# KPU-AGC/ipcr

Hardware: AMD Instinct MI355X
Metric: genome Gbases scanned/sec (k=2) (higher is better)
Workload: dtype u32

## Files before the change

### ipcr_amd/csrc/host.cpp

```cpp
#include "ipcr_hip.h"

#include <emmintrin.h>
#include <immintrin.h>
#include <sched.h>
#include <sys/prctl.h>
#include <time.h>
#include <unistd.h>
#include <dlfcn.h>
#include <hip/hip_runtime_api.h>
#include <hsa/hsa.h>
#include <hsa/hsa_ext_amd.h>

#include <algorithm>
#include <array>
#include <atomic>
#include <chrono>
#include <condition_variable>
#include <functional>
#include <cstdarg>
#include <cstdio>
#include <cstdlib>
#include <cstring>
#include <map>
#include <memory>
// ... 1788 lines not shown
        e = hipMemcpyAsync(c->d_bad, c->h_bad, 8, hipMemcpyHostToDevice, c->st);
        if (e == hipSuccess) e = hipMemcpyAsync(c->d_sites, c->h_sites, m * sizeof(ipcr_site_dev), hipMemcpyHostToDevice, c->st);
        if (e == hipSuccess) e = ipcr::launch_read_sites(c->st, g->planes, g->rst, c->d_sites, (uint32_t)m, c->d_out, g->d_exc, nruns, c->d_bad);
        if (e == hipSuccess) e = hipMemcpyAsync(out + offsets[i0], c->d_out, bytes, hipMemcpyDeviceToHost, c->st);
        if (e == hipSuccess) e = hipMemcpyAsync(c->h_bad, c->d_bad, 8, hipMemcpyDeviceToHost, c->st);
        if (e == hipSuccess) e = hipStreamSynchronize(c->st);
        if (e == hipSuccess && *c->h_bad != ~0ull) {
            const unsigned long long v = *c->h_bad;
            const int64_t i = i0 + (int64_t)(v >> 16);
            const unsigned off = (unsigned)((v >> 8) & 0xFFu), b = (unsigned)(v & 0xFFu);
            st = fail(IPCR_ERR_PRIMER, "%s: site %lld (record %d, position %lld): byte 0x%02x%s%c%s has no reverse complement "
                      "(upper-case IUPAC DNA only, core/primer/rc.go:8-24)", what, (long long)i, sites[i].record, (long long)sites[i].pos + off, b,
                      (b >= 0x21 && b < 0x7F) ? " '" : "", (b >= 0x21 && b < 0x7F) ? (char)b : ' ', (b >= 0x21 && b < 0x7F) ? "'" : "");
        }
        i0 += (int64_t)m;
    }
    read_ctx_release(c);
    if (st != IPCR_OK) return st;
    HIPCHK(e);
    return IPCR_OK;
}
}

extern "C" {

ipcr_status ipcr_genome_read_sites(const ipcr_genome *cg, const ipcr_site *sites, int64_t n, uint8_t *out, uint64_t cap,
                                   uint64_t *offsets, uint64_t *needed) {
    if (!cg || n < 0 || (n && !sites) || !offsets || !needed) return fail(IPCR_ERR_INVALID, "ipcr_genome_read_sites: null argument");
    return read_sites("ipcr_genome_read_sites", const_cast<ipcr_genome *>(cg), sites, n, out, cap, offsets, needed);
}

uint64_t ipcr_genome_exception_runs(const ipcr_genome *cg) {
    if (!cg) return 0;
    ipcr_genome *g = const_cast<ipcr_genome *>(cg);
    DeviceGuard dg(g->device);
    std::lock_guard<std::mutex> lk(g->read_mu);
    if (genome_finalize(g) != IPCR_OK) return 0;
    return (g->exc_dropped || !g->exc_capture) ? UINT64_MAX : g->exc_sorted;
}

uint32_t ipcr_genome_num_records(const ipcr_genome *g) { return g ? (uint32_t)g->rec_start.size() : 0; }
uint64_t ipcr_genome_record_len(const ipcr_genome *g, uint32_t r) { return (g && r < g->rec_len.size()) ? g->rec_len[r] : 0; }
const char *ipcr_genome_record_id(const ipcr_genome *g, uint32_t r) { return (g && r < g->ids.size()) ? g->ids[r].c_str() : ""; }
uint64_t ipcr_genome_total_bases(const ipcr_genome *g) { return g ? g->total_bases : 0; }
uint64_t ipcr_genome_tile_bytes(const ipcr_genome *g) {
    return g ? ((g->next_col + 63) / 64) * IPCR_BLOCK_PLANE_WORDS * 4ull : 0;
}
double ipcr_genome_pack_ms(const ipcr_genome *g) { return g ? g->pack_ms : 0; }

uint8_t ipcr_genome_record_flags(const ipcr_genome *g, uint32_t record) {
    if (!g || record >= g->rec_start.size()) return 0;
    if (!g->flags_valid) {
        DeviceGuard dg(g->device);
        if (genome_finalize(const_cast<ipcr_genome *>(g)) != IPCR_OK) return 0;
    }
    return (uint8_t)((g->flags[record] & 1u) | (genome_any_reset(g) ? 2u : 0u));
}

}


struct ipcr_scratch {
    const ipcr_panel *panel = nullptr;
    int device = 0;
    SetDev *sdev[2] = {nullptr, nullptr};
    hipStream_t stream = nullptr;
    hipEvent_t ev[4] = {nullptr, nullptr, nullptr, nullptr};
    ipcr_queue_entry *d_queue = nullptr;
    uint64_t qcap = 0;
    unsigned long long *d_qcounts = nullptr;
    uint64_t prefix_hint = 256;
    ipcr_hit_rec *d_hits = nullptr;
    uint64_t hcap = 0;
    unsigned long long *d_counts = nullptr;
    void *d_hitbuf = nullptr;
    uint32_t cset = 0;
    struct Lane {
        hipStream_t s = nullptr;
        ~Lane() { if (s) (void)hipStreamDestroy(s); }
    };
    std::shared_ptr<Lane> own_lane;
    std::shared_ptr<Lane> lane_next;
    std::shared_ptr<Lane> lane_used;
    hipEvent_t ev_done = nullptr;
    hipStream_t cstream = nullptr;
    struct Pending {
        bool active = false, empty = false;
        int mode = 0;
        bool fused = false;
        bool verified = false;
        bool on_lane = false;
        bool published = false;
        bool times_pending = false;
        uint32_t nrec = 0, check_rst = 0, cset_used = 0;
        uint64_t nblocks = 0, pre = 0;
        uint64_t block0 = 0;
        bool segment = false;
        std::chrono::steady_clock::time_point t0;
    } pend;
    void *pinned = nullptr;
    uint32_t *d_tickets = nullptr;
    uint32_t seq = 0;
    uint64_t seg_overflow = 0;
    std::vector<ipcr_hit> hits;
    std::vector<ipcr_hit> hits_raw;
    std::vector<uint32_t> bucket;
    std::vector<ipcr_product> products;
    std::vector<uint64_t> last_rec_len;
    std::vector<uint64_t> last_rec_start;
    ipcr_scan_stats stats{};
    std::vector<ipcr_chunk_window> windows;
    bool products_in_windows = false;
    ipcr_genome *chunk = nullptr;
    bool dev_hits_stale = false;
    bool last_was_chunk = false;
    uint8_t *h_stage[2] = {nullptr, nullptr};
    hipEvent_t ev_stage[2] = {nullptr, nullptr};
    uint8_t *h_planes = nullptr;
    uint64_t h_planes_cap = 0;
    std::shared_ptr<std::atomic<int>> counted_in;
    uint8_t *d_amps = nullptr; uint64_t amps_cap = 0;
    ipcr_genome *nest = nullptr;
    void *d_probe_misc = nullptr; uint64_t probe_misc_cap = 0;
    hipStream_t probe_stream = nullptr;
    uint8_t *h_probe = nullptr; uint64_t h_probe_cap = 0;
    uint32_t probe_tag = 0;
    hipStream_t probe_on = nullptr;
    int64_t probe_pending = -1;
    uint64_t probe_res_off = 0;
};

namespace {

constexpr uint64_t PREFIX_HITS = 65536;
constexpr uint64_t QCAP_INIT = 1ull << 13;
constexpr uint64_t HCAP_INIT = 1ull << 20;
constexpr uint64_t QCAP_MAX = 1ull << 23;
constexpr uint64_t HCAP_MAX = 1ull << 28;
uint64_t hcap_soft() {
    const char *e = getenv("IPCR_TEST_HCAP_SOFT");
    return e && *e ? std::max<uint64_t>(64, strtoull(e, nullptr, 10)) : (1ull << 24);
}

ipcr_status panel_upload(const ipcr_panel *cp, int mode, int slot, SetDev **out) {
    ipcr_panel *p = const_cast<ipcr_panel *>(cp);
    std::lock_guard<std::mutex> lock(p->mu);
    std::unique_ptr<PanelDev> &pd = p->devs[slot];
    if (!pd) { pd.reset(new PanelDev); pd->slot = slot; }
    PatternSet &s = p->set[mode];
    SetDev &d = pd->set[mode];
    *out = &d;
    if (!d.dev && !s.host.empty()) {
        HIPCHK(hipMalloc((void **)&d.dev, s.host.size() * sizeof(ipcr_dev_pattern)));
        HIPCHK(hipMemcpy(d.dev, s.host.data(), s.host.size() * sizeof(ipcr_dev_pattern), hipMemcpyHostToDevice));
    }
    const bool force_index = getenv("IPCR_FORCE_INDEX") && atoi(getenv("IPCR_FORCE_INDEX")) != 0;
    if (p->specialize && !d.jit_tried && !s.host.empty()) {
        d.jit_tried = true;
        static const bool async_on = env_flag("IPCR_JIT_ASYNC", true);
        const bool async = async_on && !force_index && s.host.size() <= 16;
        if (!force_index && !async) {
            d.jit = ipcr::jit_build(s.host, p->cfg.max_mm, s.jit_error);
            d.jit_pub.store(&d.jit, std::memory_order_release);
        } else if (async) {
            d.jit_state.store(1);
            const int max_mm = p->cfg.max_mm;
            SetDev *dp = &d;
            PatternSet *sp = &s;
            d.jit_thread = std::thread([dp, sp, max_mm, slot] {
                DeviceGuard dgt(slot);
                std::string err;
                dp->jit = ipcr::jit_build(sp->host, max_mm, err);
                if (dp->jit.empty()) sp->jit_error = err;
                dp->jit_state.store(2, std::memory_order_release);
            });
        }
// ... 167 lines not shown
    }
    dedup_sorted_hits(out);
}

void trace(const char *what, const void *s) {
    static const bool on = getenv("IPCR_DEBUG_TIMES") != nullptr;
    static const auto t0 = std::chrono::steady_clock::now();
    if (on) fprintf(stderr, "[t %10.1f us] %p %s\n", std::chrono::duration<double, std::micro>(std::chrono::steady_clock::now() - t0).count(), s, what);
}

double ms_since(std::chrono::steady_clock::time_point a) {
    return std::chrono::duration<double, std::milli>(std::chrono::steady_clock::now() - a).count();
}

bool env_flag(const char *name, bool dflt) {
    const char *v = getenv(name);
    return (v && *v) ? atoi(v) != 0 : dflt;
}

uint32_t *pinned_seq(const ipcr_scratch *s) {
    return reinterpret_cast<uint32_t *>(static_cast<char *>(s->pinned) + 64 + PREFIX_HITS * sizeof(ipcr_hit));
}

std::atomic<bool> g_publish_broken{false};

bool publish_enabled() {
    static const bool on = env_flag("IPCR_PUBLISH", true);
    return on && !g_publish_broken.load(std::memory_order_relaxed);
}

ipcr_status wait_published(ipcr_scratch *s) {
    volatile uint32_t *w = pinned_seq(s);
    const uint32_t want = s->seq;
    const hipStream_t lane = s->lane_used ? s->lane_used->s : s->stream;
    const auto t0 = std::chrono::steady_clock::now();
    static const int sleep_us = getenv("IPCR_WAIT_SLEEP_US") ? atoi(getenv("IPCR_WAIT_SLEEP_US")) : 0;
    static const int spin_us = getenv("IPCR_WAIT_SPIN_US") ? atoi(getenv("IPCR_WAIT_SPIN_US")) : 30;
    if (sleep_us > 0) {
        static thread_local bool slack_set = false;
        if (!slack_set) { (void)prctl(PR_SET_TIMERSLACK, 1000UL, 0, 0, 0); slack_set = true; }
    }
    for (uint64_t spin = 1;; ++spin) {
        if (__atomic_load_n(w, __ATOMIC_ACQUIRE) == want) return IPCR_OK;
        if (sleep_us > 0 && (spin & 63u) == 0 && ms_since(t0) * 1000.0 > (double)spin_us) {
            struct timespec ts = {0, sleep_us * 1000L};
            (void)nanosleep(&ts, nullptr);
        }
        if (spin < 0x10000u) __builtin_ia32_pause();
        else std::this_thread::yield();
        if ((spin & 0xFFFFu) == 0) {
            const hipError_t q = hipStreamQuery(lane);
            if (q == hipSuccess) {
                if (__atomic_load_n(w, __ATOMIC_ACQUIRE) == want) return IPCR_OK;
                return IPCR_ERR_UNSUPPORTED;
            }
            if (q != hipErrorNotReady) return fail(IPCR_ERR_DEVICE, "HIP: %s", hipGetErrorString(q));
            if (ms_since(t0) > 120000.0) return fail(IPCR_ERR_DEVICE, "scan did not finish within 120 s");
        }
    }
}

ipcr_status scan_segmented(const ipcr_panel *p, ipcr_scratch *s, ipcr_genome *g, uint64_t seen_hits);
inline bool hit_has_idx_below(const ipcr_hit *h, int tw);

ipcr_status scan_launch(const ipcr_panel *p, ipcr_scratch *s, ipcr_genome *g) {
    ipcr_scratch::Pending &pd = s->pend;
    const PatternSet &set = p->set[pd.mode];
    const SetDev &sd = *s->sdev[pd.mode];
    static const std::vector<ipcr::JitFilter *> none;
    const std::vector<ipcr::JitFilter *> *pub = sd.jit_pub.load(std::memory_order_acquire);
    const std::vector<ipcr::JitFilter *> &jit = pub ? *pub : none;
    const auto te = std::chrono::steady_clock::now();
    unsigned long long *cnt = s->d_counts + 4u * s->cset, *cnt_next = s->d_counts + 4u * (s->cset ^ 1u);
    const uint64_t qset = (uint64_t)IPCR_QUEUE_SHARDS * IPCR_QUEUE_COUNTER_STRIDE;
    unsigned long long *qc = s->d_qcounts + qset * s->cset, *qc_next = s->d_qcounts + qset * (s->cset ^ 1u);
    pd.cset_used = s->cset;
    s->cset ^= 1u;
    const uint64_t nblocks = pd.nblocks, block0 = pd.block0;
    trace("launch>", s);
    const hipStream_t own = s->stream;
    const hipStream_t lane = s->lane_next ? s->lane_next->s : own;
    s->lane_used = s->lane_next ? std::move(s->lane_next) : s->own_lane;
    s->lane_next.reset();
    pd.fused = false;
    pd.verified = false;
    pd.published = false;
    if (!jit.empty()) {
        ipcr::JitVerify v;
        v.rst = g->rst;
        v.pats = sd.dev;
        v.rec_start = g->d_rec_start;
        v.block_rec = g->d_block_rec;
        v.rec_len = g->d_rec_len;
        v.nrec = pd.nrec;
        v.max_mm = (uint32_t)p->cfg.max_mm;
        v.check_rst = pd.check_rst;
        v.hits = s->d_hits;
        v.hcap = s->hcap;
        v.counts = cnt;
        pd.pre = std::min<uint64_t>(PREFIX_HITS, s->hcap);
        ++s->seq;
        for (size_t gi = 0; gi < jit.size(); ++gi) {
            v.next_counts = gi == 0 ? cnt_next : nullptr;
            v.next_qcount = gi == 0 ? qc_next : nullptr;
            if (publish_enabled()) {
                v.seq = s->seq;
                v.tickets = s->d_tickets;
                v.pub_hits = reinterpret_cast<ipcr_hit_rec *>(static_cast<unsigned long long *>(s->pinned) + 8);
                v.pre = (uint32_t)pd.pre;
            }
            if (gi + 1 == jit.size() && publish_enabled()) {
                v.tickets = s->d_tickets;
                v.pub = static_cast<unsigned long long *>(s->pinned) + 4u * pd.cset_used;
                v.pub_seq = pinned_seq(s);
                static const bool break_it = env_flag("IPCR_TEST_BREAK_PUBLISH", false);
                if (break_it) v.pub_seq = s->d_tickets + 2064;
                v.seq = s->seq;
                pd.published = true;
            }
            {
                static const int withhold = [] {
                    const int w = getenv("IPCR_TEST_WITHHOLD_TAG") ? atoi(getenv("IPCR_TEST_WITHHOLD_TAG")) : 0;
                    if (w > 0) fprintf(stderr, "ipcr_hip: IPCR_TEST_WITHHOLD_TAG=%d is set: hit record %d of every scan is published torn on purpose "
                                               "(a test hook; every scan then waits out the hand-over deadline and refetches)\n", w, w - 1);
                    return w;
                }();
                v.withhold = withhold > 0 ? (uint32_t)withhold : 0u;
            }
            HIPCHK(ipcr::jit_launch(jit[gi], lane, g->planes, g->d_colmask, block0, nblocks, s->d_queue, s->qcap, qc, v,
                                    gi == 0 ? s->ev[0] : nullptr, gi + 1 == jit.size() ? s->ev[1] : nullptr));
        }
        s->stats.kernel_kind = 1;
        pd.fused = true;
    } else if (sd.index_jit) {
        const IndexPlan &ix = set.index;
        const bool more = !ix.leftover.empty();
        const bool fuse = !more && publish_enabled() && ipcr::jit_index_fusable();
        ipcr::JitVerify fv;
        if (fuse) {
            fv.rst = g->rst;
            fv.pats = sd.dev;
            fv.rec_start = g->d_rec_start;
            fv.block_rec = g->d_block_rec;
            fv.rec_len = g->d_rec_len;
            fv.nrec = pd.nrec;
            fv.max_mm = (uint32_t)p->cfg.max_mm;
            fv.check_rst = pd.check_rst;
            fv.hits = s->d_hits;
            fv.hcap = s->hcap;
            fv.counts = cnt;
            fv.next_counts = cnt_next;
            fv.next_qcount = qc_next;
            pd.pre = std::min<uint64_t>(PREFIX_HITS, s->hcap);
            ++s->seq;
            fv.seq = s->seq;
            fv.pub = static_cast<unsigned long long *>(s->pinned) + 4u * pd.cset_used;
            fv.pub_hits = reinterpret_cast<ipcr_hit_rec *>(static_cast<unsigned long long *>(s->pinned) + 8);
            fv.pre = (uint32_t)pd.pre;
            fv.pub_seq = pinned_seq(s);
            static const bool break_it = env_flag("IPCR_TEST_BREAK_PUBLISH", false);
            if (break_it) fv.pub_seq = s->d_tickets + 2064;
        }
        HIPCHK(ipcr::jit_launch_index(sd.index_jit, lane, g->planes, block0, nblocks, (uint32_t)ix.shapes.size(), sd.d_lds_image, sd.d_table,
                                      (uint32_t)p->cfg.max_mm, s->d_queue, s->qcap, qc, s->d_tickets, s->ev[0], more ? nullptr : s->ev[1],
                                      fuse ? &fv : nullptr));
        if (fuse) { pd.fused = true; pd.published = true; }
// ... 46 lines not shown

ipcr_status scan_enqueue(const ipcr_panel *p, ipcr_scratch *s, ipcr_genome *g, bool chunk = false, int chunk_reset = -1) {
    ipcr_scratch::Pending &pd = s->pend;
    if (pd.active) return fail(IPCR_ERR_INVALID, "a scan is already in flight on this scratch (ipcr_scan_genome_end not called)");
    pd.t0 = std::chrono::steady_clock::now();
    s->hits.clear();
    s->products.clear();
    s->products_in_windows = false;
    s->last_was_chunk = false;
    s->dev_hits_stale = false;
    const double pack_ms_keep = s->stats.pack_ms;
    memset(&s->stats, 0, sizeof s->stats);
    s->stats.pack_ms = pack_ms_keep;
    trace("enqueue>", s);
    ipcr_status st = chunk ? genome_finalize_async(g) : genome_finalize(g);
    if (st != IPCR_OK) return st;
    trace("finalized", s);
    s->last_rec_len = g->rec_len;
    s->last_rec_start = g->rec_start;
    const bool clean_chunks = !chunk || env_flag("IPCR_CHUNK_CLEAN_MODE", true);
    const bool any_reset = chunk ? (chunk_reset != 0 || !clean_chunks) : genome_any_reset(g);
    pd.mode = (!p->modes_equal && any_reset) ? 1 : 0;
    st = panel_upload(p, pd.mode, s->device, &s->sdev[pd.mode]);
    if (st != IPCR_OK) return st;
    const PatternSet &set = p->set[pd.mode];
    pd.nrec = (uint32_t)g->rec_start.size();
    pd.nblocks = (g->next_col + 63) / 64;
    pd.block0 = 0;
    pd.segment = false;
    pd.check_rst = any_reset ? 1u : 0u;
    s->stats.pattern_set = (uint32_t)pd.mode;
    s->stats.bases = g->total_bases;
    s->stats.tile_bytes = pd.nblocks * IPCR_BLOCK_PLANE_WORDS * 4ull;
    s->stats.n_patterns = (int32_t)set.ids.size();
    pd.empty = pd.nrec == 0 || set.ids.empty();
    pd.active = true;
    if (pd.empty) return IPCR_OK;
    st = scan_launch(p, s, g);
    if (st != IPCR_OK) pd.active = false;
    return st;
}

ipcr_status scan_collect(const ipcr_panel *p, ipcr_scratch *s, ipcr_genome *g) {
    ipcr_scratch::Pending &pd = s->pend;
    if (!pd.active) return fail(IPCR_ERR_INVALID, "no scan in flight on this scratch");
    pd.active = false;
    if (pd.empty) return IPCR_OK;
    for (int attempt = 0; attempt < 12; ++attempt) {
        const auto tw = std::chrono::steady_clock::now();
        trace("wait>", s);
        if (pd.published) {
            const ipcr_status ws = wait_published(s);
            if (ws == IPCR_ERR_UNSUPPORTED) {
                g_publish_broken.store(true);
                static std::atomic<bool> told{false};
                if (!told.exchange(true)) fprintf(stderr, "ipcr_hip: in-kernel hand-over did not reach pinned memory; using the copy path\n");
                const ipcr_status rs = scan_launch(p, s, g);
                if (rs != IPCR_OK) return rs;
                continue;
            }
            if (ws != IPCR_OK) return ws;
        } else if (pd.on_lane) HIPCHK(hipEventSynchronize(s->ev_done));
        else HIPCHK(hipStreamSynchronize(s->stream));
        s->stats.wait_ms += ms_since(tw);
        trace("wait<", s);
        const unsigned long long *pc = static_cast<unsigned long long *>(s->pinned) + 4u * pd.cset_used;
        const ipcr_hit *ph = reinterpret_cast<ipcr_hit *>(static_cast<unsigned long long *>(s->pinned) + 8);
        if (!pd.verified && pc[0] > 0) {
            const SetDev &sd = *s->sdev[pd.mode];
            if (pd.published) HIPCHK(hipEventSynchronize(s->ev[1]));
            const uint64_t qset = (uint64_t)IPCR_QUEUE_SHARDS * IPCR_QUEUE_COUNTER_STRIDE;
            unsigned long long *cnt = s->d_counts + 4u * pd.cset_used, *cnt_next = s->d_counts + 4u * (pd.cset_used ^ 1u);
            unsigned long long *qc = s->d_qcounts + qset * pd.cset_used, *qc_next = s->d_qcounts + qset * (pd.cset_used ^ 1u);
            HIPCHK(ipcr::launch_verify(s->stream, g->planes, g->rst, sd.dev, (uint32_t)p->cfg.max_mm, g->d_rec_start,
                                       g->d_rec_len, pd.nrec, pd.check_rst, s->d_queue, s->qcap, qc, s->d_hits,
                                       s->hcap, cnt + 1, cnt + 2, cnt_next, qc_next, s->ev[2], s->ev[3]));
            HIPCHK(hipMemcpyAsync(s->pinned, s->d_hitbuf, 64 + pd.pre * sizeof(ipcr_hit), hipMemcpyDeviceToHost, s->stream));
            pd.verified = true;
            pd.on_lane = false;
            pd.published = false;
            continue;
        }
        const uint64_t nhit = pc[1], ncand = pc[2], fullest = pc[3];
        if (fullest > s->qcap) {
            uint64_t want = s->qcap;
            while (want < fullest) want *= 2;
            if (want > QCAP_MAX) {
                if (p->cfg.hit_cap > 0) {
                    if (pd.segment) { s->seg_overflow = ~0ull; return IPCR_ERR_CAPACITY; }
                    return scan_segmented(p, s, g, hcap_soft() * 16u);
                }
                return fail(IPCR_ERR_CAPACITY, "%llu filter survivors in one queue segment exceed the device queue limit", (unsigned long long)fullest);
            }
            HIPCHK(hipFree(s->d_queue));
            s->d_queue = nullptr;
            HIPCHK(hipMalloc((void **)&s->d_queue, want * IPCR_QUEUE_SHARDS * sizeof(ipcr_queue_entry)));
            s->qcap = want;
            ipcr_status st = scan_launch(p, s, g);
            if (st != IPCR_OK) return st;
            continue;
        }
        if (nhit > s->hcap) {
            uint64_t want = s->hcap;
            while (want < nhit) want *= 2;
            if (p->cfg.hit_cap > 0 && nhit > hcap_soft()) {
                if (pd.segment) { s->seg_overflow = nhit; return IPCR_ERR_CAPACITY; }
                return scan_segmented(p, s, g, nhit);
            }
            if (want > HCAP_MAX) return fail(IPCR_ERR_CAPACITY, "%llu hits exceed the device hit-buffer limit", (unsigned long long)nhit);
            HIPCHK(hipFree(s->d_hitbuf));
            s->d_hitbuf = nullptr;
            s->d_hits = nullptr;
            s->d_counts = nullptr;
            HIPCHK(hipMalloc(&s->d_hitbuf, (want + 2) * sizeof(ipcr_hit_rec)));
            HIPCHK(hipMemset(s->d_hitbuf, 0, 64));
            HIPCHK(hipStreamSynchronize(nullptr));
            s->d_counts = static_cast<unsigned long long *>(s->d_hitbuf);
            s->d_hits = static_cast<ipcr_hit_rec *>(s->d_hitbuf) + 2;
            s->hcap = want;
            ipcr_status st = scan_launch(p, s, g);
            if (st != IPCR_OK) return st;
            continue;
        }
        std::vector<ipcr_hit> &raw = s->hits_raw;
        raw.resize(nhit);
        uint64_t got = std::min<uint64_t>(nhit, pd.pre);
        if (pd.published && got) {
            const volatile ipcr_hit *vh = ph;
            const uint64_t tag_pos = (uint64_t)(s->seq & 0xFFFFFFu);
            const uint64_t tag_hi = (uint64_t)s->seq << 32;
            bool complete = true;
            const auto tw0 = std::chrono::steady_clock::now();
            for (uint64_t i = 0; i < got && complete; ++i) {
                for (uint64_t spin = 1; (vh[i].pos >> 40) != tag_pos || vh[i].mm_mask[1] != (tag_hi | (uint32_t)i); ++spin) {
                    __builtin_ia32_pause();
                    if ((spin & 0xFFFu) == 0 && ms_since(tw0) > 2.0) { complete = false; break; }
                }
            }
            std::atomic_thread_fence(std::memory_order_acquire);
            if (!complete) {
                ++s->stats.handover_refetched;
                HIPCHK(hipEventSynchronize(s->ev[1]));
                if (!s->cstream) HIPCHK(hipStreamCreateWithFlags(&s->cstream, hipStreamNonBlocking));
                HIPCHK(hipMemcpyAsync(raw.data(), s->d_hits, got * sizeof(ipcr_hit), hipMemcpyDeviceToHost, s->cstream));
                HIPCHK(hipStreamSynchronize(s->cstream));
            } else {
                memcpy(raw.data(), ph, got * sizeof(ipcr_hit));
                for (uint64_t i = 0; i < got; ++i) {
                    raw[i].pos &= (1ull << 40) - 1ull;
                    raw[i].mm_mask[1] = 0;
                }
            }
        } else if (got) {
            memcpy(raw.data(), ph, got * sizeof(ipcr_hit));
        }
        if (pd.published) HIPCHK(hipEventSynchronize(s->ev[1]));
        if (nhit > got) HIPCHK(hipMemcpy(raw.data() + got, s->d_hits + got, (nhit - got) * sizeof(ipcr_hit), hipMemcpyDeviceToHost));
        s->prefix_hint = std::max<uint64_t>(256, nhit + nhit / 4 + 16);
        float fms = 0, vms = 0;
        static const bool check_pub = env_flag("IPCR_DEBUG_PUBLISH_CHECK", false);
        if (check_pub && pd.published && got) {
            std::vector<ipcr_hit> dev(got);
            HIPCHK(hipMemcpy(dev.data(), s->d_hits, got * sizeof(ipcr_hit), hipMemcpyDeviceToHost));
            uint64_t diff = 0;
            for (uint64_t i = 0; i < got; ++i)
                if (memcmp(&dev[i], &raw[i], sizeof(ipcr_hit)) != 0) ++diff;
            s->stats.handover_check_diffs += diff;
            ++s->stats.handover_checked;
            if (diff) fprintf(stderr, "publish check: %llu of %llu hit records taken from pinned memory differ from device memory\n",
                              (unsigned long long)diff, (unsigned long long)got);
        }
        trace("retired", s);
        HIPCHK(hipEventElapsedTime(&fms, s->ev[0], s->ev[1]));
        if (pd.verified) HIPCHK(hipEventElapsedTime(&vms, s->ev[2], s->ev[3]));
        s->stats.filter_ms = fms;
        s->stats.verify_ms = vms;
        s->stats.candidates = ncand;
        s->stats.hits = nhit;
        const auto ts = std::chrono::steady_clock::now();
        sort_hits(raw, s->hits, pd.nrec, (uint32_t)p->defs.size());
        s->stats.sort_ms = ms_since(ts);
        s->stats.total_ms = ms_since(pd.t0);
        trace("sorted", s);
        return IPCR_OK;
    }
    return fail(IPCR_ERR_CAPACITY, "scan buffers kept overflowing");
}

ipcr_status scan_segmented(const ipcr_panel *p, ipcr_scratch *s, ipcr_genome *g, uint64_t seen_hits) {
    ipcr_scratch::Pending &pd = s->pend;
    const uint64_t total = (g->next_col + 63) / 64;
    const uint64_t cap = (uint64_t)p->cfg.hit_cap;
    const size_t ndefs = p->defs.size();
    std::vector<ipcr_hit> kept;
    std::map<uint64_t, uint64_t> passed;
    uint64_t seg = std::max<uint64_t>(1, total * (hcap_soft() / 2) / std::max<uint64_t>(seen_hits, 1));
    double filter_ms = 0, verify_ms = 0;
    uint64_t cand = 0;
    for (uint64_t b0 = 0; b0 < total;) {
        const uint64_t nb = std::min(seg, total - b0);
        pd.active = true;
        pd.segment = true;
        pd.block0 = b0;
        pd.nblocks = nb;
        ipcr_status st = scan_launch(p, s, g);
        if (st == IPCR_OK) st = scan_collect(p, s, g);
        if (st == IPCR_ERR_CAPACITY && s->seg_overflow) {
            s->seg_overflow = 0;
            if (seg == 1) return fail(IPCR_ERR_CAPACITY, "one block of the genome holds more raw matches than the device hit buffer may take");
            seg = std::max<uint64_t>(1, nb / 2);
            continue;
        }
        if (st != IPCR_OK) return st;
        filter_ms += s->stats.filter_ms;
        verify_ms += s->stats.verify_ms;
        cand += s->stats.candidates;
        for (const ipcr_hit &h : s->hits) {
            const uint32_t pat = h.pattern & 0x7FFFFFFFu;
            uint64_t &n = passed[((uint64_t)h.record << 32) | pat];
            if (n >= cap) continue;
            kept.push_back(h);
            const bool dropped_by_host = pat < ndefs && p->defs[pat].left && hit_has_idx_below(&h, p->tw);
            if (!dropped_by_host) ++n;
        }
        b0 += nb;
    }
    pd.segment = false;
    pd.block0 = 0;
    pd.nblocks = total;
    s->hits_raw = kept;
    sort_hits(s->hits_raw, s->hits, pd.nrec, (uint32_t)ndefs);
    s->stats.filter_ms = filter_ms;
    s->stats.verify_ms = verify_ms;
    s->stats.candidates = cand;
    s->stats.hits = s->hits.size();
    s->stats.segmented = 1;
    s->dev_hits_stale = true;
    s->stats.total_ms = ms_since(pd.t0);
    return IPCR_OK;
}

ipcr_status scan_hits(const ipcr_panel *p, ipcr_scratch *s, ipcr_genome *g) {
    ipcr_status st = scan_enqueue(p, s, g);
    if (st != IPCR_OK) return st;
    return scan_collect(p, s, g);
}

struct MatchRef {
    int64_t pos;
    const ipcr_hit *h;
};

inline int hit_mm(const ipcr_hit *h) { return __builtin_popcountll(h->mm_mask[0]) + __builtin_popcountll(h->mm_mask[1]); }

inline bool hit_has_idx_below(const ipcr_hit *h, int tw) {
    if (tw <= 0) return false;
// ... 186 lines not shown
ipcr_status join_sorted_hits(const ipcr_panel *p, ipcr_scratch *s, const uint64_t *rec_len, const uint8_t *rec_flags,
                             uint32_t nrec, ipcr_emit_fn emit, void *user) {
    const std::vector<ipcr_hit> &H = s->hits;
    struct Range { size_t i, j; uint32_t rec; };
    std::vector<Range> ranges;
    for (size_t i = 0; i < H.size();) {
        const uint32_t rec = H[i].record;
        size_t j = i;
        while (j < H.size() && H[j].record == rec) ++j;
        if (rec >= nrec) return fail(IPCR_ERR_INVALID, "hit refers to record %u of %u", rec, nrec);
        ranges.push_back({i, j, rec});
        i = j;
    }
    const bool par_env = env_flag("IPCR_JOIN_PARALLEL", true);
    if (par_env && ranges.size() > 1 && H.size() >= 32768 && PackPool::get().size() > 1) {
        std::vector<std::vector<ipcr_product>> outs(ranges.size());
        PackPool::get().run(ranges.size(), [&](size_t r) {
            JoinCtx c{p, &outs[r], nullptr, nullptr};
            const Range &g = ranges[r];
            (void)join_one_record(p, H, g.i, g.j, g.rec, (int64_t)rec_len[g.rec], rec_flags ? rec_flags[g.rec] : 0, c);
        });
        for (const auto &o : outs)
            for (const ipcr_product &pr : o) {
                s->products.push_back(pr);
                if (emit && emit(&s->products.back(), user) != 0) return fail(IPCR_ERR_ABORTED, "emit callback aborted the scan");
            }
    } else {
        JoinCtx c{p, &s->products, emit, user};
        for (const Range &g : ranges)
            if (!join_one_record(p, H, g.i, g.j, g.rec, (int64_t)rec_len[g.rec], rec_flags ? rec_flags[g.rec] : 0, c))
                return fail(IPCR_ERR_ABORTED, "emit callback aborted the scan");
    }
    s->stats.products = s->products.size();
    return IPCR_OK;
}

ipcr_status scratch_ready(const ipcr_panel *p, ipcr_scratch *s, bool need_device = true) {
    if (!p || !s) return fail(IPCR_ERR_INVALID, "null panel or scratch");
    if (s->panel != p) return fail(IPCR_ERR_INVALID, "scratch was created for a different panel");
    if (need_device && !s->stream) return fail(IPCR_ERR_DEVICE, "host-only scratch cannot scan: the ipcr scan path has no CPU fallback");
    return IPCR_OK;
}

ipcr_status same_device(const ipcr_scratch *s, const ipcr_genome *g) {
    if (!g) return fail(IPCR_ERR_INVALID, "null genome");
    if (s->stream && s->device != g->device)
        return fail(IPCR_ERR_INVALID, "scratch lives on device %d, the genome on device %d: scan a genome with a scratch of its own device (ipcr_scratch_create_on)", s->device, g->device);
    return IPCR_OK;
}

}

extern "C" {

ipcr_status ipcr_scratch_create(const ipcr_panel *p, ipcr_scratch **out) {
    return ipcr_scratch_create_on(p, default_slot(), out);
}

int32_t ipcr_scratch_device(const ipcr_scratch *s) { return (s && s->stream) ? s->device : -1; }

ipcr_status ipcr_scratch_create_on(const ipcr_panel *p, int32_t device, ipcr_scratch **out) {
    if (!p || !out) return fail(IPCR_ERR_INVALID, "ipcr_scratch_create: null argument");
    *out = nullptr;
    if (slot_count() == 0) return fail(IPCR_ERR_DEVICE, "no HIP device visible: the ipcr scan path has no CPU fallback");
    if (device < 0 || device >= slot_count()) return fail(IPCR_ERR_INVALID, "ipcr_scratch_create_on: device %d of %d", device, slot_count());
    DeviceGuard dg(device);
    std::unique_ptr<ipcr_scratch> s(new ipcr_scratch);
    s->panel = p;
    ipcr_scratch *raw = s.get();
    auto build = [&]() -> ipcr_status {
        raw->device = device;
        raw->own_lane = std::make_shared<ipcr_scratch::Lane>();
        {
            static const int lane_prio = env_flag("IPCR_LANE_PRIORITY", false) ? 1 : 0;
            if (lane_prio) {
                int lo = 0, hi = 0;
                HIPCHK(hipDeviceGetStreamPriorityRange(&lo, &hi));
                HIPCHK(hipStreamCreateWithPriority(&raw->own_lane->s, hipStreamNonBlocking, hi));
            } else {
                HIPCHK(hipStreamCreateWithFlags(&raw->own_lane->s, hipStreamNonBlocking));
            }
        }
        raw->stream = raw->own_lane->s;
        for (auto &e : raw->ev) HIPCHK(hipEventCreate(&e));
        raw->qcap = QCAP_INIT;
        raw->hcap = HCAP_INIT;
        HIPCHK(hipMalloc((void **)&raw->d_queue, raw->qcap * IPCR_QUEUE_SHARDS * sizeof(ipcr_queue_entry)));
        HIPCHK(hipMalloc((void **)&raw->d_qcounts, 2ull * IPCR_QUEUE_SHARDS * IPCR_QUEUE_COUNTER_STRIDE * 8ull));
        HIPCHK(hipMemset(raw->d_qcounts, 0, 2ull * IPCR_QUEUE_SHARDS * IPCR_QUEUE_COUNTER_STRIDE * 8ull));
        HIPCHK(hipMalloc(&raw->d_hitbuf, (raw->hcap + 2) * sizeof(ipcr_hit_rec)));
        HIPCHK(hipMemset(raw->d_hitbuf, 0, 64));
        raw->d_counts = static_cast<unsigned long long *>(raw->d_hitbuf);
        raw->d_hits = static_cast<ipcr_hit_rec *>(raw->d_hitbuf) + 2;
        HIPCHK(hipHostMalloc(&raw->pinned, 64 + PREFIX_HITS * sizeof(ipcr_hit) + 64, hipHostMallocDefault));
        memset(raw->pinned, 0, 64 + PREFIX_HITS * sizeof(ipcr_hit) + 64);
        HIPCHK(hipMalloc((void **)&raw->d_tickets, 65 * 128));
        HIPCHK(hipMemset(raw->d_tickets, 0, 65 * 128));
        HIPCHK(hipStreamSynchronize(nullptr));
        raw->counted_in = p->live_scratches;
        raw->counted_in->fetch_add(1);
        return IPCR_OK;
    };
    ipcr_status st = build();
    if (st != IPCR_OK) { ipcr_scratch_destroy(s.release()); return st; }
    *out = s.release();
    return IPCR_OK;
}

ipcr_status ipcr_scratch_create_host(const ipcr_panel *p, ipcr_scratch **out) {
    if (!p || !out) return fail(IPCR_ERR_INVALID, "ipcr_scratch_create_host: null argument");
    ipcr_scratch *s = new ipcr_scratch;
    s->panel = p;
    *out = s;
    return IPCR_OK;
}

void ipcr_scratch_destroy(ipcr_scratch *s) {
    if (!s) return;
    DeviceGuard dg(s->device);
    if (s->stream) {
        if (s->pend.active && s->lane_used) (void)hipStreamSynchronize(s->lane_used->s);
        (void)hipStreamSynchronize(s->stream);
    }
    if (s->counted_in) s->counted_in->fetch_sub(1);
    for (int h = 0; h < 2; ++h) {
        if (s->h_stage[h]) (void)hipHostFree(s->h_stage[h]);
        if (s->ev_stage[h]) (void)hipEventDestroy(s->ev_stage[h]);
        if (h == 0 && s->h_planes) (void)hipHostFree(s->h_planes);
    }
    if (s->chunk) ipcr_genome_destroy(s->chunk);
    if (s->nest) ipcr_genome_destroy(s->nest);
    if (s->d_queue) (void)hipFree(s->d_queue);
    if (s->d_qcounts) (void)hipFree(s->d_qcounts);
    if (s->d_hitbuf) (void)hipFree(s->d_hitbuf);
    if (s->d_amps) (void)hipFree(s->d_amps);
    if (s->d_probe_misc) (void)hipFree(s->d_probe_misc);
    if (s->pinned) (void)hipHostFree(s->pinned);
    if (s->d_tickets) (void)hipFree(s->d_tickets);
    for (auto &e : s->ev)
        if (e) (void)hipEventDestroy(e);
    if (s->ev_done) (void)hipEventDestroy(s->ev_done);
    if (s->cstream) (void)hipStreamDestroy(s->cstream);
    if (s->probe_stream) (void)hipStreamDestroy(s->probe_stream);
    if (s->h_probe) (void)hipHostFree(s->h_probe);
    delete s;
}

ipcr_status ipcr_scratch_stats(const ipcr_scratch *s, ipcr_scan_stats *out) {
    if (!s || !out) return fail(IPCR_ERR_INVALID, "null argument");
    *out = s->stats;
    return IPCR_OK;
}

ipcr_status ipcr_scratch_products(const ipcr_scratch *s, const ipcr_product **out, int64_t *n) {
    if (!s || !out || !n) return fail(IPCR_ERR_INVALID, "null argument");
    *out = s->products.data();
    *n = (int64_t)s->products.size();
    return IPCR_OK;
}

ipcr_status ipcr_scratch_hits(const ipcr_scratch *s, const ipcr_hit **out, int64_t *n) {
    if (!s || !out || !n) return fail(IPCR_ERR_INVALID, "null argument");
    *out = s->hits.data();
    *n = (int64_t)s->hits.size();
    return IPCR_OK;
}

ipcr_status ipcr_scratch_device_hits(const ipcr_scratch *s, const void **dev_block, uint64_t *n_hits, uint64_t *capacity) {
    if (!s || !dev_block || !n_hits || !capacity) return fail(IPCR_ERR_INVALID, "null argument");
    if (!s->d_hitbuf) return fail(IPCR_ERR_DEVICE, "host-only scratch has no device hit buffer");
    *dev_block = s->d_hitbuf;
    *n_hits = s->hits_raw.size();
    *capacity = s->hcap;
    if (s->dev_hits_stale)
        return fail(IPCR_ERR_UNSUPPORTED, "the device hit buffer does not hold this scan's hits: a capped scan that ran in segments keeps them on the host "
                                          "(ipcr_scratch_hits; ipcr_exchange_begin sends them from there)");
    return IPCR_OK;
}

}
ipcr_status ipcr_internal_scratch_send_block(const ipcr_scratch *s, const void **dev_block, uint64_t *hcap, const ipcr_hit **host_hits,
                                             uint64_t *n_host, int *authoritative) {
    if (!s || !s->d_hitbuf) return fail(IPCR_ERR_DEVICE, "host-only scratch has no device hit buffer");
    *dev_block = s->d_hitbuf;
    *hcap = s->hcap;
    *host_hits = s->hits_raw.data();
    *n_host = s->hits_raw.size();
    *authoritative = s->dev_hits_stale ? 0 : 1;
    return IPCR_OK;
}
extern "C" {

ipcr_status ipcr_scan_genome_hits(const ipcr_panel *p, ipcr_scratch *s, const ipcr_genome *g) {
    ipcr_status st = scratch_ready(p, s);
    if (st == IPCR_OK) st = same_device(s, g);
    if (st != IPCR_OK) return st;
    DeviceGuard dg(s->device);
    s->stats.pack_ms = 0;
    return scan_hits(p, s, const_cast<ipcr_genome *>(g));
}

ipcr_status ipcr_scan_genome(const ipcr_panel *p, ipcr_scratch *s, const ipcr_genome *g, ipcr_emit_fn emit, void *user) {
    const auto t0 = std::chrono::steady_clock::now();
    ipcr_status st = ipcr_scan_genome_hits(p, s, g);
    if (st != IPCR_OK) return st;
    std::vector<uint8_t> fl(g->rec_start.size());
    const bool any = genome_any_reset(g);
    for (size_t r = 0; r < fl.size(); ++r) fl[r] = (uint8_t)((g->flags[r] & 1u) | (any ? 2u : 0u));
    const auto tj = std::chrono::steady_clock::now();
    st = join_sorted_hits(p, s, g->rec_len.data(), fl.data(), (uint32_t)fl.size(), emit, user);
    s->stats.join_ms = std::chrono::duration<double, std::milli>(std::chrono::steady_clock::now() - tj).count();
    s->stats.total_ms = std::chrono::duration<double, std::milli>(std::chrono::steady_clock::now() - t0).count();
    return st;
}

static void record_windows(uint32_t rec, uint64_t len, int64_t chunk, int64_t step, std::vector<ipcr_chunk_window> &out) {
    uint64_t ws = 0, last_end = 0;
    bool emitted = false;
    if (step > 0)
        while (len - ws > (uint64_t)chunk) {
            out.push_back({rec, 0u, ws, ws + (uint64_t)chunk, 0u, 0u});
            last_end = ws + (uint64_t)chunk;
            emitted = true;
// ... 34 lines not shown
    if (chunk_size <= 0 || step <= 0) step = 0;
    const uint32_t nrec = (uint32_t)g->rec_start.size();
    s->windows.clear();
    std::vector<size_t> first_window(nrec + 1, 0);
    for (uint32_t r = 0; r < nrec; ++r) {
        first_window[r] = s->windows.size();
        record_windows(r, g->rec_len[r], chunk_size, step, s->windows);
    }
    first_window[nrec] = s->windows.size();
    {
        std::vector<uint64_t> ab;
        std::vector<size_t> which;
        for (size_t w = 0; w < s->windows.size(); ++w) {
            const ipcr_chunk_window &cw = s->windows[w];
            if (!(g->flags[cw.record] & 1u) || cw.end <= cw.start) continue;
            ab.push_back(g->rec_start[cw.record] + cw.start);
            ab.push_back(g->rec_start[cw.record] + cw.end);
            which.push_back(w);
        }
        if (!which.empty()) {
            uint64_t *d_ab = nullptr;
            uint32_t *d_fl = nullptr;
            std::vector<uint32_t> fl(which.size(), 0);
            HIPCHK(hipMalloc((void **)&d_ab, ab.size() * 8u + which.size() * 4u));
            d_fl = reinterpret_cast<uint32_t *>(d_ab + ab.size());
            hipError_t e = hipMemcpyAsync(d_ab, ab.data(), ab.size() * 8u, hipMemcpyHostToDevice, s->stream);
            if (e == hipSuccess) e = ipcr::launch_window_reset(s->stream, g->rst, d_ab, (uint32_t)which.size(), d_fl);
            if (e == hipSuccess) e = hipMemcpyAsync(fl.data(), d_fl, which.size() * 4u, hipMemcpyDeviceToHost, s->stream);
            if (e == hipSuccess) e = hipStreamSynchronize(s->stream);
            (void)hipFree(d_ab);
            if (e != hipSuccess) return fail(IPCR_ERR_DEVICE, "HIP: %s (window reset flags)", hipGetErrorString(e));
            for (size_t i = 0; i < which.size(); ++i) s->windows[which[i]].reset = fl[i] ? 1u : 0u;
        }
    }
    const auto tj = std::chrono::steady_clock::now();
    const bool mode1 = s->pend.mode == 1;
    const std::vector<ipcr_hit> &H = s->hits;
    std::vector<ipcr_hit> wh;
    std::vector<uint32_t> by_pos;
    JoinCtx c{p, &s->products, emit, user};
    size_t i = 0;
    for (uint32_t r = 0; r < nrec && !c.aborted; ++r) {
        while (i < H.size() && H[i].record < r) ++i;
        size_t j = i;
        while (j < H.size() && H[j].record == r) ++j;
        by_pos.resize(j - i);
        for (size_t h = i; h < j; ++h) by_pos[h - i] = (uint32_t)(h - i);
        std::sort(by_pos.begin(), by_pos.end(), [&](uint32_t a, uint32_t b) { return H[i + a].pos != H[i + b].pos ? H[i + a].pos < H[i + b].pos : a < b; });
        size_t lo = 0;
        for (size_t w = first_window[r]; w < first_window[r + 1] && !c.aborted; ++w) {
            const ipcr_chunk_window &cw = s->windows[w];
            wh.clear();
            while (lo < by_pos.size() && H[i + by_pos[lo]].pos < cw.start) ++lo;
            for (size_t q = lo; q < by_pos.size() && H[i + by_pos[q]].pos < cw.end; ++q) {
                const ipcr_hit &hh = H[i + by_pos[q]];
                const uint32_t gid = hh.pattern & 0x7FFFFFFFu;
                const uint64_t L = gid < p->defs.size() ? p->defs[gid].seq.size() : 0;
                if (hh.pos + L > cw.end) continue;
                wh.push_back(hh);
                wh.back().pos -= cw.start;
                wh.back().record = (uint32_t)w;
            }
            if (wh.empty()) continue;
            std::sort(wh.begin(), wh.end(), HitLess());
            const uint8_t fl = (uint8_t)((cw.reset ? 1u : 0u) | (mode1 ? 2u : 0u));
            (void)join_one_record(p, wh, 0, wh.size(), (uint32_t)w, (int64_t)(cw.end - cw.start), fl, c);
        }
        i = j;
    }
    s->stats.products = s->products.size();
    s->products_in_windows = true;
    s->stats.join_ms = std::chrono::duration<double, std::milli>(std::chrono::steady_clock::now() - tj).count();
    s->stats.total_ms = std::chrono::duration<double, std::milli>(std::chrono::steady_clock::now() - t0).count();
    if (c.aborted) return fail(IPCR_ERR_ABORTED, "emit callback aborted the scan");
    return IPCR_OK;
}

ipcr_status ipcr_scratch_chain_after(ipcr_scratch *s, const ipcr_scratch *prev) {
    if (!s || !prev) return fail(IPCR_ERR_INVALID, "ipcr_scratch_chain_after: null argument");
    if (!s->stream || !prev->stream) return fail(IPCR_ERR_DEVICE, "host-only scratch cannot scan");
    if (s == prev) return fail(IPCR_ERR_INVALID, "ipcr_scratch_chain_after: a scratch cannot follow itself");
    if (s->pend.active) return fail(IPCR_ERR_INVALID, "ipcr_scratch_chain_after: a scan is in flight on this scratch");
    if (s->device != prev->device) return fail(IPCR_ERR_INVALID, "ipcr_scratch_chain_after: scratches of different devices");
    s->lane_next = prev->lane_used ? prev->lane_used : prev->own_lane;
    return IPCR_OK;
}

ipcr_status ipcr_scan_genome_begin(const ipcr_panel *p, ipcr_scratch *s, const ipcr_genome *g) {
    ipcr_status st = scratch_ready(p, s);
    if (st == IPCR_OK) st = same_device(s, g);
    if (st != IPCR_OK) return st;
    DeviceGuard dg(s->device);
    s->stats.pack_ms = 0;
    return scan_enqueue(p, s, const_cast<ipcr_genome *>(g));
}

ipcr_status ipcr_scan_genome_end(const ipcr_panel *p, ipcr_scratch *s, const ipcr_genome *g, ipcr_emit_fn emit, void *user) {
    ipcr_status st = scratch_ready(p, s);
    if (st == IPCR_OK) st = same_device(s, g);
    if (st != IPCR_OK) return st;
    DeviceGuard dg(s->device);
    st = scan_collect(p, s, const_cast<ipcr_genome *>(g));
    if (st != IPCR_OK) return st;
    std::vector<uint8_t> fl(g->rec_start.size());
    const bool any = genome_any_reset(g);
    for (size_t r = 0; r < fl.size(); ++r) fl[r] = (uint8_t)((g->flags[r] & 1u) | (any ? 2u : 0u));
    const auto tj = std::chrono::steady_clock::now();
    st = join_sorted_hits(p, s, g->rec_len.data(), fl.data(), (uint32_t)fl.size(), emit, user);
    s->stats.join_ms = std::chrono::duration<double, std::milli>(std::chrono::steady_clock::now() - tj).count();
    s->stats.total_ms = std::chrono::duration<double, std::milli>(std::chrono::steady_clock::now() - s->pend.t0).count();
    trace("joined", s);
    return st;
}

ipcr_status ipcr_join_hits(const ipcr_panel *p, ipcr_scratch *s, const ipcr_hit *hits, int64_t n_hits,
                           const uint64_t *record_len, const uint8_t *record_flags, uint32_t n_records,
                           ipcr_emit_fn emit, void *user) {
    ipcr_status st = scratch_ready(p, s, false);
    if (st != IPCR_OK) return st;
    if ((n_hits > 0 && !hits) || (n_records > 0 && !record_len) || n_hits < 0) return fail(IPCR_ERR_INVALID, "ipcr_join_hits: null argument");
    s->hits_raw.assign(hits, hits + n_hits);
    sort_hits(s->hits_raw, s->hits, n_records, (uint32_t)p->defs.size());
    s->products.clear();
    s->products_in_windows = false;
    s->last_was_chunk = false;
    return join_sorted_hits(p, s, record_len, record_flags, n_records, emit, user);
}

static void stream_copy(uint8_t *dst, const uint8_t *src, uint64_t n) {
    static const bool plain = getenv("IPCR_CHUNK_NTCOPY") && atoi(getenv("IPCR_CHUNK_NTCOPY")) == 0;
    uint64_t i = 0;
    if (!plain && (reinterpret_cast<uintptr_t>(dst) & 15u) == 0) {
        for (; i + 64 <= n; i += 64) {
            const __m128i a = _mm_loadu_si128(reinterpret_cast<const __m128i *>(src + i));
            const __m128i b = _mm_loadu_si128(reinterpret_cast<const __m128i *>(src + i + 16));
            const __m128i c = _mm_loadu_si128(reinterpret_cast<const __m128i *>(src + i + 32));
            const __m128i d = _mm_loadu_si128(reinterpret_cast<const __m128i *>(src + i + 48));
            _mm_stream_si128(reinterpret_cast<__m128i *>(dst + i), a);
            _mm_stream_si128(reinterpret_cast<__m128i *>(dst + i + 16), b);
            _mm_stream_si128(reinterpret_cast<__m128i *>(dst + i + 32), c);
            _mm_stream_si128(reinterpret_cast<__m128i *>(dst + i + 48), d);
        }
        _mm_sfence();
    }
    if (i < n) memcpy(dst + i, src + i, n - i);
}

ipcr_status ipcr_scan_chunk(const ipcr_panel *p, ipcr_scratch *s, const uint8_t *seq, uint64_t len,
                            ipcr_emit_fn emit, void *user) {
    const auto t0 = std::chrono::steady_clock::now();
    ipcr_status st = scratch_ready(p, s);
    if (st != IPCR_OK) return st;
    if (!seq && len) return fail(IPCR_ERR_INVALID, "null sequence");
    s->hits.clear();
    s->products.clear();
    s->products_in_windows = false;
    memset(&s->stats, 0, sizeof s->stats);
    s->last_was_chunk = p->id.empty();
    if (p->id.empty()) return IPCR_OK;
    DeviceGuard dg(s->device);
    const uint64_t need_cols = record_cols(len) + 64;
    if (!s->chunk || s->chunk->cap_cols < need_cols) {
        if (s->chunk) ipcr_genome_destroy(s->chunk);
        s->chunk = nullptr;
        st = ipcr_genome_create_on((need_cols + (need_cols >> 2)) * IPCR_COLUMN_BASES, 1, s->device, &s->chunk);
        if (st != IPCR_OK) return st;
        s->chunk->exc_capture = false;
        (void)hipStreamDestroy(s->chunk->stream);
        s->chunk->stream = s->stream;
// ... 777 lines not shown
```

Baseline: 19740.

## Alternate chained scratches across two stream lanes and correct overlapped filter timing

Chained scratches now alternate between two stream lanes instead of all serializing on the predecessor's lane, so consecutive scans can run concurrently on the device. The old single lane stays available through the IPCR_CHAIN_LANES<=1 environment setting. Start/stop events move into pooled, reference-counted sweep-event objects that track a frontier, so each scan's reported filter time subtracts the part that overlapped its predecessor. This adds event pooling, extra synchronization before queue or hit-buffer regrowth, and a per-call environment lookup for the debug publish check.

```diff
diff --git a/ipcr_amd/csrc/host.cpp b/ipcr_amd/csrc/host.cpp
--- a/ipcr_amd/csrc/host.cpp
+++ b/ipcr_amd/csrc/host.cpp
@@ -1894,6 +1894,19 @@
     std::shared_ptr<Lane> own_lane;
     std::shared_ptr<Lane> lane_next;
     std::shared_ptr<Lane> lane_used;
+    std::shared_ptr<Lane> lane_other_next;
+    std::shared_ptr<Lane> lane_other;
+    struct SweepEv {
+        hipEvent_t start = nullptr, stop = nullptr;
+        std::shared_ptr<SweepEv> frontier;
+        ~SweepEv() {
+            if (start) (void)hipEventDestroy(start);
+            if (stop) (void)hipEventDestroy(stop);
+        }
+    };
+    std::vector<std::shared_ptr<SweepEv>> sweep_evs;
+    std::shared_ptr<SweepEv> sweep_ev;
+    std::shared_ptr<SweepEv> pred_next;
     hipEvent_t ev_done = nullptr;
     hipStream_t cstream = nullptr;
     struct Pending {
@@ -1904,6 +1917,7 @@
         bool on_lane = false;
         bool published = false;
         bool times_pending = false;
+        std::shared_ptr<SweepEv> pred;
         uint32_t nrec = 0, check_rst = 0, cset_used = 0;
         uint64_t nblocks = 0, pre = 0;
         uint64_t block0 = 0;
@@ -2237,6 +2251,25 @@
     const hipStream_t lane = s->lane_next ? s->lane_next->s : own;
     s->lane_used = s->lane_next ? std::move(s->lane_next) : s->own_lane;
     s->lane_next.reset();
+    s->lane_other = std::move(s->lane_other_next);
+    s->lane_other_next.reset();
+    pd.pred = std::move(s->pred_next);
+    s->pred_next.reset();
+    {
+        s->sweep_ev.reset();
+        for (const auto &e : s->sweep_evs)
+            if (e.use_count() == 1) { s->sweep_ev = e; break; }
+        if (!s->sweep_ev) {
+            auto e = std::make_shared<ipcr_scratch::SweepEv>();
+            HIPCHK(hipEventCreate(&e->start));
+            HIPCHK(hipEventCreate(&e->stop));
+            s->sweep_evs.push_back(e);
+            s->sweep_ev = std::move(e);
+        }
+        s->sweep_ev->frontier.reset();
+        s->ev[0] = s->sweep_ev->start;
+        s->ev[1] = s->sweep_ev->stop;
+    }
     pd.fused = false;
     pd.verified = false;
     pd.published = false;
@@ -2449,6 +2482,7 @@
             continue;
         }
         const uint64_t nhit = pc[1], ncand = pc[2], fullest = pc[3];
+        if ((fullest > s->qcap || nhit > s->hcap) && pd.published) HIPCHK(hipEventSynchronize(s->ev[1]));
         if (fullest > s->qcap) {
             uint64_t want = s->qcap;
             while (want < fullest) want *= 2;
@@ -2525,7 +2559,7 @@
         if (nhit > got) HIPCHK(hipMemcpy(raw.data() + got, s->d_hits + got, (nhit - got) * sizeof(ipcr_hit), hipMemcpyDeviceToHost));
         s->prefix_hint = std::max<uint64_t>(256, nhit + nhit / 4 + 16);
         float fms = 0, vms = 0;
-        static const bool check_pub = env_flag("IPCR_DEBUG_PUBLISH_CHECK", false);
+        const bool check_pub = env_flag("IPCR_DEBUG_PUBLISH_CHECK", false);
         if (check_pub && pd.published && got) {
             std::vector<ipcr_hit> dev(got);
             HIPCHK(hipMemcpy(dev.data(), s->d_hits, got * sizeof(ipcr_hit), hipMemcpyDeviceToHost));
@@ -2539,6 +2573,20 @@
         }
         trace("retired", s);
         HIPCHK(hipEventElapsedTime(&fms, s->ev[0], s->ev[1]));
+        if (pd.pred) {
+            const std::shared_ptr<ipcr_scratch::SweepEv> front = pd.pred->frontier ? pd.pred->frontier : pd.pred;
+            HIPCHK(hipEventSynchronize(front->stop));
+            float lead = 0;
+            if (hipEventElapsedTime(&lead, s->ev[0], front->stop) != hipSuccess) {
+                (void)hipGetLastError();
+                lead = 0;
+            }
+            if (lead >= fms) {
+                fms = 0;
+                s->sweep_ev->frontier = front;
+            } else if (lead > 0) fms -= lead;
+            pd.pred.reset();
+        }
         if (pd.verified) HIPCHK(hipEventElapsedTime(&vms, s->ev[2], s->ev[3]));
         s->stats.filter_ms = fms;
         s->stats.verify_ms = vms;
@@ -2891,7 +2939,8 @@
             }
         }
         raw->stream = raw->own_lane->s;
-        for (auto &e : raw->ev) HIPCHK(hipEventCreate(&e));
+        HIPCHK(hipEventCreate(&raw->ev[2]));
+        HIPCHK(hipEventCreate(&raw->ev[3]));
         raw->qcap = QCAP_INIT;
         raw->hcap = HCAP_INIT;
         HIPCHK(hipMalloc((void **)&raw->d_queue, raw->qcap * IPCR_QUEUE_SHARDS * sizeof(ipcr_queue_entry)));
@@ -2946,8 +2995,8 @@
     if (s->d_probe_misc) (void)hipFree(s->d_probe_misc);
     if (s->pinned) (void)hipHostFree(s->pinned);
     if (s->d_tickets) (void)hipFree(s->d_tickets);
-    for (auto &e : s->ev)
-        if (e) (void)hipEventDestroy(e);
+    for (int e = 2; e < 4; ++e)
+        if (s->ev[e]) (void)hipEventDestroy(s->ev[e]);
     if (s->ev_done) (void)hipEventDestroy(s->ev_done);
     if (s->cstream) (void)hipStreamDestroy(s->cstream);
     if (s->probe_stream) (void)hipStreamDestroy(s->probe_stream);
@@ -3148,9 +3197,21 @@
     if (s == prev) return fail(IPCR_ERR_INVALID, "ipcr_scratch_chain_after: a scratch cannot follow itself");
     if (s->pend.active) return fail(IPCR_ERR_INVALID, "ipcr_scratch_chain_after: a scan is in flight on this scratch");
     if (s->device != prev->device) return fail(IPCR_ERR_INVALID, "ipcr_scratch_chain_after: scratches of different devices");
-    s->lane_next = prev->lane_used ? prev->lane_used : prev->own_lane;
-    return IPCR_OK;
-}
+    const std::shared_ptr<ipcr_scratch::Lane> &prev_lane = prev->lane_used ? prev->lane_used : prev->own_lane;
+    const char *lv = getenv("IPCR_CHAIN_LANES");
+    if (lv && *lv && atoi(lv) <= 1) {
+        s->lane_next = prev_lane;
+        s->lane_other_next.reset();
+        s->pred_next.reset();
+        return IPCR_OK;
+    }
+    s->lane_next = prev->lane_other ? prev->lane_other : s->own_lane;
+    s->lane_other_next = prev_lane;
+    s->pred_next = s->lane_next != prev_lane ? prev->sweep_ev : nullptr;
+    return IPCR_OK;
+}
+
+void *ipcr_internal_scratch_lane(const ipcr_scratch *s) { return (s && s->lane_used) ? (void *)s->lane_used->s : nullptr; }
 
 ipcr_status ipcr_scan_genome_begin(const ipcr_panel *p, ipcr_scratch *s, const ipcr_genome *g) {
     ipcr_status st = scratch_ready(p, s);
```

Result: faster. 21440 (median of 6 runs) (+8.6%).
